# RockingMat/Prot2Text-V2-esm3

Hardware: AMD Instinct MI355X
Metric: contrastive-step samples/sec (protein-text pairs) (higher is better)
Workload: dtype bf16; 1 GPU; cfg3: esm2_t36_3B + Llama-3.1-8B-Instruct (text layers 1-16), per-GPU batch 16 x 1024 residues / 16 x 128 text tokens, readout mix, InfoNCE tau=0.05, adapter fwd+bwd + clip + AdamW, train mode (dropout 0.3), segments 1; global_batch=16, parallelism=dp1 (single process, no collective), streams=text tower and encoder segments on separate HIP streams

## Files before the change

### prot2text-v2-esm3_amd/csrc/gemm_mfma.hip

```cpp
#include <atomic>
#include <type_traits>

#include "common.h"
#include "epilogue.h"
#include "gemm_tile_common.h"
#include "kernels.h"

namespace p2t {

typedef __bf16 bf16x8 __attribute__((ext_vector_type(8)));
using gptr_t = const __attribute__((address_space(1))) void*;
using lptr_t = __attribute__((address_space(3))) void*;

template <int MT, typename Epi, int MODE = TILE_FULL>
__device__ __forceinline__ void gemm_tile(char* smem, const bf16_t* __restrict__ A, int64_t lda, const bf16_t* __restrict__ W,
                                          int64_t ldw, int64_t M, int N, int k0, int ns, int64_t m0, int n0, int n_cover,
                                          const EpiParams& ep, const SplitFix* fix = nullptr, int fix_tile = 0) {
    constexpr int WN = 4, NT = 4, BM = 2 * MT * 16, BN = 256;
    constexpr int AI = BM / 128;
    constexpr int SLOT = (BM + BN) * 64;

    const int lane = threadIdx.x & 63;
    const int w = __builtin_amdgcn_readfirstlane(threadIdx.x >> 6);
    const int wm = w / WN, wn = w % WN;
// ... 333 lines not shown
            tile_coords(n_items + t, n_items + n_tail, tiles_m, tiles_n, tm, tn);
            gemm_tile<8, Epi, TILE_CONSUME>(smem, A, lda, W, ldw, M, N, 0, ns0, (int64_t)tm * 256, tn * 256, n_cover, ep, &fix, t);
        }
    }
}

template <typename Epi>
__global__ void __launch_bounds__(512)
    gemm_nt_mfma_tail_kernel(const bf16_t* __restrict__ A, int64_t lda, const bf16_t* __restrict__ W, int64_t ldw, int64_t M,
                             int N, int K, int tiles_m, int tiles_n, int n_full, int n_tail, int n_cover, EpiParams ep,
                             SplitFix fix) {
    __shared__ __attribute__((aligned(16))) char smem[4 * 512 * 64];
    const int bid = blockIdx.x, ns = K >> 5, ns0 = (ns >> 1) & ~1;
    int tm, tn;
    if (bid < n_full) {
        tile_coords(bid, n_full + n_tail, tiles_m, tiles_n, tm, tn);
        gemm_tile<8, Epi>(smem, A, lda, W, ldw, M, N, 0, ns, (int64_t)tm * 256, tn * 256, n_cover, ep);
    } else if (bid < n_full + n_tail) {
        const int t = bid - n_full;
        tile_coords(n_full + t, n_full + n_tail, tiles_m, tiles_n, tm, tn);
        gemm_tile<8, Epi, TILE_PRODUCE>(smem, A, lda, W, ldw, M, N, ns0 * 32, ns - ns0, (int64_t)tm * 256, tn * 256, n_cover, ep, &fix, t);
    } else {
        const int t = bid - n_full - n_tail;
        tile_coords(n_full + t, n_full + n_tail, tiles_m, tiles_n, tm, tn);
        gemm_tile<8, Epi, TILE_CONSUME>(smem, A, lda, W, ldw, M, N, 0, ns0, (int64_t)tm * 256, tn * 256, n_cover, ep, &fix, t);
    }
}

template <typename Epi>
int launch_gemm_w4_persist(const void* A, int64_t lda, const void* W, int64_t ldw, int64_t M, int N, int K, int n_items, int n_tail, int grid,
                           const EpiParams& ep, const SplitFix& fix, hipStream_t s, int sched = 1);
int launch_gemm_w4(const void* A, int64_t lda, const void* W, int64_t ldw, int64_t M, int N, int K, int n_cover, int out_dtype, int epilogue,
                   const EpiParams& ep, hipStream_t s);
template <typename Epi>
int launch_gemm_w4_pairs(const void* A, int64_t lda, const void* W, int64_t ldw, int64_t M, int N, int K, int n_tail, const EpiParams& ep,
                         const SplitFix& fix, hipStream_t s);
template <typename Epi>
constexpr bool kHasW4Pairs = std::is_same<Epi, EpiResid>::value || std::is_same<Epi, EpiStore<bf16_t>>::value || std::is_same<Epi, EpiStore<float>>::value;
template <typename Epi>
constexpr bool kHasW4 = std::is_same<Epi, EpiStore<bf16_t>>::value || std::is_same<Epi, EpiStore<float>>::value || std::is_same<Epi, EpiResid>::value ||
                        std::is_same<Epi, EpiQkvRope<bf16_t>>::value || std::is_same<Epi, EpiGelu<bf16_t>>::value || std::is_same<Epi, EpiSwiglu<bf16_t>>::value;
template <typename Epi>
constexpr int kW4TileCode = std::is_same<Epi, EpiStore<bf16_t>>::value || std::is_same<Epi, EpiStore<float>>::value ? P2T_EPI_STORE
                            : std::is_same<Epi, EpiResid>::value                                                     ? P2T_EPI_RESID
                            : std::is_same<Epi, EpiGelu<bf16_t>>::value                                              ? P2T_EPI_GELU
                            : std::is_same<Epi, EpiQkvRope<bf16_t>>::value                                           ? P2T_EPI_QKV_ROPE
                                                                                                                      : -1;
template <typename Epi>
constexpr int kW4TileOut = std::is_same<Epi, EpiResid>::value || std::is_same<Epi, EpiStore<float>>::value ? P2T_F32 : P2T_BF16;

struct EpiTraits {
    bool rmw;
    bool w4;
    bool w4_pairs;
    bool w4_tile;
};
template <typename Epi>
constexpr EpiTraits kEpiTraits = {Epi::kRmw, kHasW4<Epi>, kHasW4Pairs<Epi>,
                                  std::is_same<Epi, EpiQkvRope<bf16_t>>::value || std::is_same<Epi, EpiStore<bf16_t>>::value};

GemmFacts gemm_facts(int64_t M, int N, int K, int n_cover, int64_t lda, int64_t ldw, int cus, size_t fix_bytes) {
    GemmFacts f;
    f.M = M; f.lda = lda; f.ldw = ldw; f.N = N; f.K = K; f.n_cover = n_cover; f.cus = cus; f.fix_bytes = fix_bytes;
    f.ns = K >> 5;
    f.tn = ceil_div(n_cover, 256);
    f.items = ceil_div(M, 256) * f.tn;
    f.rem = f.items % cus;
    f.whole_tiles = M % 256 == 0 && N % 256 == 0 && n_cover == N;
    f.stride32 = (int64_t)256 * (lda > ldw ? lda : ldw) * 2 < ((int64_t)1 << 32);
    return f;
}

bool small_tiles_pay(const GemmFacts& f) {
    const double cost256 = (double)ceil_div(f.items, f.cus);
    const double cost128 = (double)ceil_div(ceil_div(f.M, 128) * f.tn, f.cus) * 0.625 * 1.08;
    return cost256 > cost128;
}

static std::atomic<int> g_gemm_policy{0};
void set_gemm_policy(int policy) { g_gemm_policy.store(policy, std::memory_order_relaxed); }
int get_gemm_policy() { return g_gemm_policy.load(std::memory_order_relaxed); }

constexpr size_t kFixHeader = 2048, kFixSlab = 256 * 256 * sizeof(float);
size_t gemm_fix_workspace_bytes() { return kFixHeader + 128 * kFixSlab; }
size_t gemm_fix_header_bytes() { return kFixHeader; }

static bool fix_fits(const GemmFacts& f, int64_t n_tiles) { return f.fix_bytes >= kFixHeader + (size_t)n_tiles * kFixSlab; }

static SplitFix split_fix(void* fix_ws, unsigned fix_epoch) {
    SplitFix f{};
    f.flag = (unsigned*)fix_ws;
    f.timeout = fault_word_ptr();
    f.slab = (float*)((char*)fix_ws + kFixHeader);
    f.epoch = fix_epoch;
    return f;
}


static bool persist_fits(const GemmFacts& f) { return f.whole_tiles && f.items >= f.cus && (f.ns & 3) == 0 && f.ns >= 12; }

static bool persist_pays(const GemmFacts& f, const EpiTraits& t) {
    return persist_fits(f) && (f.rem == 0 || f.ns >= 128 || f.items >= 4 * f.cus || t.rmw);
}

static GemmPlan persist8(const GemmFacts& f, bool pairs, bool halves) {
    GemmPlan p{GEMM_PERSIST, f.cus, f.items};
    if (f.rem == 0 || 2 * f.rem > f.cus || f.rem > 128) return p;
    pairs = pairs && (f.ns & 7) == 0 && fix_fits(f, f.rem);
    if (pairs || halves) {
        p.n_full = f.items - f.rem;
        p.n_tail = f.rem;
        p.half_tail = !pairs;
    }
    return p;
}

static GemmPlan persist4(const GemmFacts& f, bool pairs, int sched = 1) {
    const int64_t t = pairs && f.rem > 0 && 2 * f.rem <= f.cus && fix_fits(f, f.rem) ? f.rem : 0;
    const int64_t n = f.items - t;
    return {GEMM_W4_PERSIST, n < f.cus ? n : f.cus, n, t, 0, sched};
}

static GemmPlan per_tile8(const GemmFacts& f, bool rows128) {
    const int64_t g = rows128 ? ceil_div(f.M, 128) * f.tn : f.items;
    return {rows128 ? GEMM_TILE128 : GEMM_TILE256, g, g};
}

static bool pairs_pay(const GemmFacts& f) { return f.ns >= 192; }

static GemmPlan plan_persist(const GemmFacts& f, const EpiTraits& t, bool no_w4) {
    if (t.w4 && !no_w4 && f.stride32) return persist4(f, pairs_pay(f));
    return persist8(f, pairs_pay(f), true);
}

static GemmPlan plan_per_tile(const GemmFacts& f, const EpiTraits& t, bool no_w4) {
    const int64_t items = f.items;
    if (t.w4_tile && !no_w4 && f.whole_tiles && items < f.cus && items * 4 >= f.cus * 3 && f.K % 128 == 0 && f.K >= 256 && f.stride32)
        return {GEMM_W4_TILE, items, items};
    const bool half_round_long_k = items * 2 <= f.cus && items * 8 >= f.cus * 3 && f.K >= 8192 && fix_fits(f, items);
    if (t.w4_pairs && !no_w4 && f.whole_tiles && half_round_long_k && f.K % 128 == 0 && f.stride32) return {GEMM_W4_PAIRS, 2 * items, 0, items};
    if (half_round_long_k) return {GEMM_SPLITK, 2 * items, 0, items};
    if (small_tiles_pay(f)) return per_tile8(f, true);
    const int64_t n_full = (items / f.cus) * f.cus, n_tail = items - n_full;
    if (n_full > 0 && n_tail > 0 && n_tail <= 128 && (f.ns >= 128 || (f.ns >= 64 && n_full >= 4 * f.cus)) && fix_fits(f, n_tail))
        return {GEMM_SPLITK, n_full + 2 * n_tail, n_full, n_tail};
    return per_tile8(f, false);
}

static GemmPlan plan_default(const GemmFacts& f, const EpiTraits& t, bool no_w4) {
    return persist_pays(f, t) ? plan_persist(f, t, no_w4) : plan_per_tile(f, t, no_w4);
}

#ifdef P2T_LAB
#include "../../tools/lab/gemm_forms_lab.h"
#endif

template <typename Epi>
static GemmPlan plan_shape(const GemmFacts& f, int policy) {
#ifdef P2T_LAB
    if (policy != 0 && policy != 9) return plan_lab<Epi>(f, policy);
#endif
    return plan_default(f, kEpiTraits<Epi>, policy == 9);
}

static int policy_cus() {
#ifdef P2T_LAB
// ... 92 lines not shown
```

### prot2text-v2-esm3_amd/csrc/gemm_tile_common.h

```cpp
#pragma once
#include "common.h"
#include <type_traits>

#include "epilogue.h"

namespace p2t {

struct SplitFix {
    float* slab;
    unsigned* flag;
    unsigned* timeout;
    unsigned epoch;
};
enum { TILE_FULL = 0, TILE_PRODUCE = 1, TILE_CONSUME = 2 };


__device__ __forceinline__ void tile_coords(int id, int n_items, int tiles_m, int tiles_n, int& tm, int& tn) {
    const int q8 = n_items >> 3, r8 = n_items & 7, xcd = id & 7;
    const int swz_id = (xcd < r8 ? xcd * (q8 + 1) : r8 * (q8 + 1) + (xcd - r8) * q8) + (id >> 3);
    constexpr int GM = 4;
    const int band = swz_id / (GM * tiles_n), first_m = band * GM;
    const int gm = min(GM, tiles_m - first_m);
    const int in_band = swz_id - band * GM * tiles_n;
    tm = first_m + in_band % gm;
    tn = in_band / gm;
}

template <int MT, typename Epi, bool INTERIOR = false, bool ADD = false>
__device__ __forceinline__ void tile_epilogue(const f32x4 (&acc)[4][MT], const EpiParams& ep, int64_t M, int N, int n_cover,
                                              int64_t m0, int n0, int wm, int wn, int fr, int kg, const float4* addend = nullptr,
                                              int add_stride = 0, float poison = 0.f) {
    const int nb = n0 + wn * 64 + kg * 8;
    if (!INTERIOR && nb >= n_cover) return;
    float b0[8], b1[8];
#pragma unroll
    for (int e = 0; e < 8; ++e) b0[e] = b1[e] = 0.f;
    if (ep.bias) {
        if (INTERIOR || nb < N) loadW<8>(ep.bias + nb, b0);
        if (INTERIOR || nb + 32 < N) loadW<8>(ep.bias + nb + 32, b1);
    }
    if constexpr (INTERIOR && Epi::kRmw && MT % 4 == 0 && !ADD) {
#pragma unroll
        for (int jb = 0; jb < MT; jb += 4) {
            float r0[4][8], r1[4][8];
#pragma unroll
            for (int jj = 0; jj < 4; ++jj) Epi::template fetch2<8>(ep, m0 + wm * MT * 16 + (jb + jj) * 16 + fr, nb, r0[jj], r1[jj]);
#pragma unroll
            for (int jj = 0; jj < 4; ++jj) {
                const int j = jb + jj;
                const float v0[8] = {acc[0][j][0], acc[0][j][1], acc[0][j][2], acc[0][j][3], acc[1][j][0], acc[1][j][1], acc[1][j][2], acc[1][j][3]};
                const float v1[8] = {acc[2][j][0], acc[2][j][1], acc[2][j][2], acc[2][j][3], acc[3][j][0], acc[3][j][1], acc[3][j][2], acc[3][j][3]};
                Epi::template apply2_fetched<8>(ep, m0 + wm * MT * 16 + j * 16 + fr, nb, v0, v1, b0, b1, r0[jj], r1[jj]);
            }
        }
    } else {
#pragma unroll
        for (int j = 0; j < MT; ++j) {
            const int64_t m = m0 + wm * MT * 16 + j * 16 + fr;
            if (!INTERIOR && m >= M) continue;
            float v0[8] = {acc[0][j][0], acc[0][j][1], acc[0][j][2], acc[0][j][3], acc[1][j][0], acc[1][j][1], acc[1][j][2], acc[1][j][3]};
            float v1[8] = {acc[2][j][0], acc[2][j][1], acc[2][j][2], acc[2][j][3], acc[3][j][0], acc[3][j][1], acc[3][j][2], acc[3][j][3]};
            if constexpr (ADD) {
                const float4 p0 = addend[(0 * MT + j) * add_stride], p1 = addend[(1 * MT + j) * add_stride];
                const float4 p2 = addend[(2 * MT + j) * add_stride], p3 = addend[(3 * MT + j) * add_stride];
                v0[0] += p0.x + poison; v0[1] += p0.y + poison; v0[2] += p0.z + poison; v0[3] += p0.w + poison;
                v0[4] += p1.x + poison; v0[5] += p1.y + poison; v0[6] += p1.z + poison; v0[7] += p1.w + poison;
                v1[0] += p2.x + poison; v1[1] += p2.y + poison; v1[2] += p2.z + poison; v1[3] += p2.w + poison;
                v1[4] += p3.x + poison; v1[5] += p3.y + poison; v1[6] += p3.z + poison; v1[7] += p3.w + poison;
            }
            Epi::template apply2<8, INTERIOR>(ep, m, nb, v0, v1, b0, b1);
        }
    }
}

template <typename Epi, typename = void> struct epi_has_fetch_shared : std::false_type {};
template <typename Epi> struct epi_has_fetch_shared<Epi, std::void_t<decltype(&Epi::fetch_shared)>> : std::true_type {};
template <typename Epi, typename = void> struct epi_has_fetch : std::false_type {};
template <typename Epi> struct epi_has_fetch<Epi, std::void_t<decltype(Epi::kFetch)>> : std::true_type {};
#define P2T_EPI_PIN_GROUP(h, j) \
    asm volatile("" : "+a"(acc[h][0][j]), "+a"(acc[h][1][j]), "+a"(acc[h][2][j]), "+a"(acc[h][3][j])::"memory");
template <int MT, typename Epi, int P = 4>
__device__ __forceinline__ void tile_epilogue_pair(f32x4 (&acc)[2][4][MT], const EpiParams& ep, int64_t m0, int n0, int wm, int wn, int fr, int kg) {
    const int nb0 = n0 + wn * 128 + kg * 8;
    float b[2][2][8];
#pragma unroll
    for (int h = 0; h < 2; ++h)
#pragma unroll
        for (int e = 0; e < 8; ++e) b[h][0][e] = b[h][1][e] = 0.f;
    if (ep.bias) {
#pragma unroll
        for (int h = 0; h < 2; ++h) {
            loadW<8>(ep.bias + nb0 + h * 64, b[h][0]);
            loadW<8>(ep.bias + nb0 + h * 64 + 32, b[h][1]);
        }
    }
    const int64_t mrow = m0 + wm * MT * 16 + fr;
    if constexpr (epi_has_fetch_shared<Epi>::value && P > 0) {
        if (Epi::fetch_shared(ep)) {
            constexpr int PS = P < MT ? P : MT;
            float r[PS][2][8];
#pragma unroll
            for (int u = 0; u < PS; ++u)
#pragma unroll
                for (int e = 0; e < 8; ++e) r[u][0][e] = r[u][1][e] = 0.f;
#pragma unroll
            for (int u = 0; u < PS; ++u) Epi::template fetch2<8, true>(ep, mrow + u * 16, nb0, r[u][0], r[u][1]);
            __builtin_amdgcn_sched_barrier(0);
#pragma unroll
            for (int u = 0; u < MT; ++u) {
                float s0[8], s1[8];
#pragma unroll
                for (int e = 0; e < 8; ++e) { s0[e] = r[u % PS][0][e]; s1[e] = r[u % PS][1][e]; }
                __builtin_amdgcn_sched_barrier(0);
                if (u + PS < MT) Epi::template fetch2<8, true>(ep, mrow + (u + PS) * 16, nb0, r[u % PS][0], r[u % PS][1]);
                __builtin_amdgcn_sched_barrier(0);
#pragma unroll
                for (int h = 0; h < 2; ++h) {
                    P2T_EPI_PIN_GROUP(h, u)
                    const float v0[8] = {acc[h][0][u][0], acc[h][0][u][1], acc[h][0][u][2], acc[h][0][u][3], acc[h][1][u][0], acc[h][1][u][1], acc[h][1][u][2], acc[h][1][u][3]};
                    const float v1[8] = {acc[h][2][u][0], acc[h][2][u][1], acc[h][2][u][2], acc[h][2][u][3], acc[h][3][u][0], acc[h][3][u][1], acc[h][3][u][2], acc[h][3][u][3]};
                    Epi::template apply2_fetched<8, true>(ep, mrow + u * 16, nb0 + h * 64, v0, v1, b[h][0], b[h][1], s0, s1);
                    __builtin_amdgcn_sched_barrier(0);
                }
            }
            return;
        }
    }
    if constexpr ((Epi::kRmw || epi_has_fetch<Epi>::value) && P > 0) {
        constexpr int G = 2 * MT;
        float r[P][2][8];
        if constexpr (!Epi::kRmw) {
#pragma unroll
            for (int g = 0; g < P; ++g)
#pragma unroll
                for (int e = 0; e < 8; ++e) r[g][0][e] = r[g][1][e] = 0.f;
        }
#pragma unroll
        for (int g = 0; g < P; ++g) Epi::template fetch2<8, true>(ep, mrow + (g % MT) * 16, nb0 + (g / MT) * 64, r[g][0], r[g][1]);
        __builtin_amdgcn_sched_barrier(0);
#pragma unroll
        for (int g = 0; g < G; ++g) {
            const int h = g / MT, j = g % MT;
            P2T_EPI_PIN_GROUP(h, j)
            const float v0[8] = {acc[h][0][j][0], acc[h][0][j][1], acc[h][0][j][2], acc[h][0][j][3], acc[h][1][j][0], acc[h][1][j][1], acc[h][1][j][2], acc[h][1][j][3]};
            const float v1[8] = {acc[h][2][j][0], acc[h][2][j][1], acc[h][2][j][2], acc[h][2][j][3], acc[h][3][j][0], acc[h][3][j][1], acc[h][3][j][2], acc[h][3][j][3]};
            float s0[8], s1[8];
#pragma unroll
            for (int e = 0; e < 8; ++e) { s0[e] = r[g % P][0][e]; s1[e] = r[g % P][1][e]; }
            __builtin_amdgcn_sched_barrier(0);
            if (g + P < G) Epi::template fetch2<8, true>(ep, mrow + ((g + P) % MT) * 16, nb0 + ((g + P) / MT) * 64, r[g % P][0], r[g % P][1]);
            __builtin_amdgcn_sched_barrier(0);
            Epi::template apply2_fetched<8, true>(ep, mrow + j * 16, nb0 + h * 64, v0, v1, b[h][0], b[h][1], s0, s1);
            __builtin_amdgcn_sched_barrier(0);
        }
    } else {
#pragma unroll
        for (int h = 0; h < 2; ++h)
#pragma unroll
            for (int j = 0; j < MT; ++j) {
                P2T_EPI_PIN_GROUP(h, j)
                const float v0[8] = {acc[h][0][j][0], acc[h][0][j][1], acc[h][0][j][2], acc[h][0][j][3], acc[h][1][j][0], acc[h][1][j][1], acc[h][1][j][2], acc[h][1][j][3]};
                const float v1[8] = {acc[h][2][j][0], acc[h][2][j][1], acc[h][2][j][2], acc[h][2][j][3], acc[h][3][j][0], acc[h][3][j][1], acc[h][3][j][2], acc[h][3][j][3]};
                Epi::template apply2<8, true>(ep, mrow + j * 16, nb0 + h * 64, v0, v1, b[h][0], b[h][1]);
                __builtin_amdgcn_sched_barrier(0);
            }
    }
}

}
```

### prot2text-v2-esm3_amd/csrc/gemm_w4.hip

```cpp
#include <type_traits>

#include "common.h"
#include "epilogue.h"
#include "gemm_tile_common.h"
#include "kernels.h"

namespace p2t {
#ifdef P2T_LAB
__device__ uint64_t* g_lab_stamp_ptr = nullptr;
#endif

typedef __bf16 bf16x8 __attribute__((ext_vector_type(8)));

template <typename Epi, bool PERSIST, int SCHED = 1, bool PAIRS_ONLY = false>
__global__ void __launch_bounds__(256)
    gemm_nt_w4_kernel(const bf16_t* __restrict__ A, int64_t lda, const bf16_t* __restrict__ W, int64_t ldw, int64_t M, int N, int K,
                      int tiles_m, int tiles_n, int n_items, int n_tail, int n_cover, EpiParams ep, SplitFix fix) {
    constexpr int MT = 8, NT = 8, BUF = 512 * 128, WOFF = 256 * 128, NL = 16;
#ifndef P2T_LAB
    static_assert(SCHED == 1, "the product library carries one instruction order of the K loop; order 0 is in the lab build");
#endif
    constexpr int kEpiOps = 2 * MT * Epi::kMinOps;
    constexpr int kIssuedBeforeWait = SCHED == 0 ? 6 : 9;
    constexpr int kExtCount = kIssuedBeforeWait + kEpiOps > 63 ? 63 : kIssuedBeforeWait + kEpiOps;
// ... 102 lines not shown
            P2T_W4_R0W(0) P2T_W4_PAIR(F, wb, xb, 4) P2T_W4_R0W(1) P2T_W4_PAIR(F, wb, xb, 5) P2T_W4_R0X(0) P2T_W4_GPAIR(9, F, wb, xb, 6) P2T_W4_R0W(2) P2T_W4_PAIR(F, wb, xb, 7)
            P2T_W4_R0W(3) P2T_W4_PAIR(F, wb, xb, 8) P2T_W4_R0X(1) P2T_W4_GPAIR(10, F, wb, xb, 9) P2T_W4_R0W(4) P2T_W4_PAIR(F, wb, xb, 10) P2T_W4_R0W(5) P2T_W4_PAIR(F, wb, xb, 11)
            P2T_W4_R0X(2) P2T_W4_GPAIR(11, F, wb, xb, 12) P2T_W4_R0W(6) P2T_W4_PAIR(F, wb, xb, 13) P2T_W4_R0W(7) P2T_W4_PAIR(F, wb, xb, 14) P2T_W4_R0X(3) P2T_W4_GPAIR(12, F, wb, xb, 15)
            P2T_W4_R0X(4) P2T_W4_PAIR(F, wb, xb, 16) P2T_W4_R0X(5) P2T_W4_PAIR(F, wb, xb, 17) P2T_W4_R0X(6) P2T_W4_GPAIR(13, F, wb, xb, 18) P2T_W4_R0X(7) P2T_W4_PAIR(F, wb, xb, 19)
            P2T_W4_PAIR(F, wb, xb, 20) P2T_W4_GPAIR(14, F, wb, xb, 21) P2T_W4_PAIR(F, wb, xb, 22) P2T_W4_PAIR(F, wb, xb, 23)
            P2T_W4_GPAIR(15, F, wb, xb, 24) P2T_W4_PAIR(F, wb, xb, 25) P2T_W4_PAIR(F, wb, xb, 26) P2T_W4_PAIR(F, wb, xb, 27)
            P2T_W4_PAIR(F, wb, xb, 28) P2T_W4_PAIR(F, wb, xb, 29) P2T_W4_PAIR(F, wb, xb, 30) P2T_W4_PAIR(F, wb, xb, 31)
        }
#ifdef P2T_LAB
        else if constexpr (SCHED == 0) {
            P2T_W4_R1W(0) P2T_W4_PAIR(FI, wa, xa, 0) P2T_W4_R1W(1) P2T_W4_PAIR(FI, wa, xa, 1) P2T_W4_R1X(0) P2T_W4_PAIR(FI, wa, xa, 2) P2T_W4_R1W(2) P2T_W4_PAIR(FI, wa, xa, 3)
            P2T_W4_R1W(3) P2T_W4_PAIR(FI, wa, xa, 4) P2T_W4_R1X(1) P2T_W4_PAIR(FI, wa, xa, 5) P2T_W4_R1W(4) P2T_W4_PAIR(FI, wa, xa, 6) P2T_W4_R1W(5) P2T_W4_PAIR(FI, wa, xa, 7)
            P2T_W4_R1X(2) P2T_W4_PAIR(FI, wa, xa, 8) P2T_W4_R1W(6) P2T_W4_PAIR(FI, wa, xa, 9) P2T_W4_R1W(7) P2T_W4_PAIR(FI, wa, xa, 10) P2T_W4_R1X(3) P2T_W4_PAIR(FI, wa, xa, 11)
            P2T_W4_R1X(4) P2T_W4_PAIR(FI, wa, xa, 12) P2T_W4_R1X(5) P2T_W4_PAIR(FI, wa, xa, 13) P2T_W4_R1X(6) P2T_W4_PAIR(FI, wa, xa, 14) P2T_W4_R1X(7) P2T_W4_PAIR(FI, wa, xa, 15)
            P2T_W4_PAIR(FI, wa, xa, 16) P2T_W4_PAIR(FI, wa, xa, 17) P2T_W4_PAIR(FI, wa, xa, 18) P2T_W4_PAIR(FI, wa, xa, 19)
            asm volatile("s_waitcnt lgkmcnt(0)\n\ts_barrier" ::: "memory");
            P2T_W4_GPAIR(0, FI, wa, xa, 20) P2T_W4_PAIR(FI, wa, xa, 21) P2T_W4_GPAIR(1, FI, wa, xa, 22) P2T_W4_PAIR(FI, wa, xa, 23)
            P2T_W4_PAIR(FI, wa, xa, 24) P2T_W4_GPAIR(2, FI, wa, xa, 25) P2T_W4_PAIR(FI, wa, xa, 26) P2T_W4_PAIR(FI, wa, xa, 27)
            P2T_W4_GPAIR(3, FI, wa, xa, 28) P2T_W4_PAIR(FI, wa, xa, 29) P2T_W4_PAIR(FI, wa, xa, 30) P2T_W4_GPAIR(4, FI, wa, xa, 31)
            P2T_W4_PAIR(F, wb, xb, 0) P2T_W4_GPAIR(5, F, wb, xb, 1) P2T_W4_PAIR(F, wb, xb, 2) P2T_W4_PAIR(F, wb, xb, 3)
            P2T_W4_WAIT_NEXT_STAGE
            P2T_W4_R0W(0) P2T_W4_GPAIR(6, F, wb, xb, 4) P2T_W4_R0W(1) P2T_W4_PAIR(F, wb, xb, 5) P2T_W4_R0X(0) P2T_W4_PAIR(F, wb, xb, 6) P2T_W4_R0W(2) P2T_W4_GPAIR(7, F, wb, xb, 7)
            P2T_W4_R0W(3) P2T_W4_PAIR(F, wb, xb, 8) P2T_W4_R0X(1) P2T_W4_PAIR(F, wb, xb, 9) P2T_W4_R0W(4) P2T_W4_GPAIR(8, F, wb, xb, 10) P2T_W4_R0W(5) P2T_W4_PAIR(F, wb, xb, 11)
            P2T_W4_R0X(2) P2T_W4_PAIR(F, wb, xb, 12) P2T_W4_R0W(6) P2T_W4_GPAIR(9, F, wb, xb, 13) P2T_W4_R0W(7) P2T_W4_PAIR(F, wb, xb, 14) P2T_W4_R0X(3) P2T_W4_PAIR(F, wb, xb, 15)
            P2T_W4_R0X(4) P2T_W4_GPAIR(10, F, wb, xb, 16) P2T_W4_R0X(5) P2T_W4_PAIR(F, wb, xb, 17) P2T_W4_R0X(6) P2T_W4_PAIR(F, wb, xb, 18) P2T_W4_R0X(7) P2T_W4_GPAIR(11, F, wb, xb, 19)
            P2T_W4_PAIR(F, wb, xb, 20) P2T_W4_PAIR(F, wb, xb, 21) P2T_W4_GPAIR(12, F, wb, xb, 22) P2T_W4_PAIR(F, wb, xb, 23)
            P2T_W4_PAIR(F, wb, xb, 24) P2T_W4_GPAIR(13, F, wb, xb, 25) P2T_W4_PAIR(F, wb, xb, 26) P2T_W4_PAIR(F, wb, xb, 27)
            P2T_W4_GPAIR(14, F, wb, xb, 28) P2T_W4_PAIR(F, wb, xb, 29) P2T_W4_PAIR(F, wb, xb, 30) P2T_W4_GPAIR(15, F, wb, xb, 31)
        }
#endif
        a_ptr += 128; w_ptr += 128;
#undef P2T_W4_WAIT_NEXT_STAGE
#undef P2T_W4_PAIR
#undef P2T_W4_R1W
#undef P2T_W4_R1X
#undef P2T_W4_R0W
#undef P2T_W4_R0X
#undef P2T_W4_G
#undef P2T_W4_GPAIR
        asm volatile("s_waitcnt lgkmcnt(0)" ::: "memory");
    };
    using I0 = std::integral_constant<int, 0>;
    using I1 = std::integral_constant<int, 1>;

    auto prologue = [&]() {
#pragma unroll
    for (int b = 0; b < 2; ++b) {
#pragma unroll
        for (int q = 0; q < NL; ++q) dma1(q, b);
        a_ptr += 128; w_ptr += 128;
    }
    asm volatile("s_waitcnt vmcnt(%0)\n\ts_barrier" ::"n"(NL) : "memory");
    rd(wa[0], w_addr, std::integral_constant<int, 0>{}); rd(wa[1], w_addr, std::integral_constant<int, 2048>{});
    rd(wa[2], w_addr, std::integral_constant<int, 4096>{}); rd(wa[3], w_addr, std::integral_constant<int, 6144>{});
    rd(wa[4], w_addr, std::integral_constant<int, 8192>{}); rd(wa[5], w_addr, std::integral_constant<int, 10240>{});
    rd(wa[6], w_addr, std::integral_constant<int, 12288>{}); rd(wa[7], w_addr, std::integral_constant<int, 14336>{});
    rd(xa[0], x_addr, std::integral_constant<int, 0>{}); rd(xa[1], x_addr, std::integral_constant<int, 2048>{});
    rd(xa[2], x_addr, std::integral_constant<int, 4096>{}); rd(xa[3], x_addr, std::integral_constant<int, 6144>{});
    rd(xa[4], x_addr, std::integral_constant<int, 8192>{}); rd(xa[5], x_addr, std::integral_constant<int, 10240>{});
    rd(xa[6], x_addr, std::integral_constant<int, 12288>{}); rd(xa[7], x_addr, std::integral_constant<int, 14336>{});
    asm volatile("s_waitcnt lgkmcnt(0)" ::: "memory");
    };
    auto k_loop = [&](f32x4 (&acc)[2][4][MT], int nk_l, bool ext, bool has_next, int64_t nm0, int nn0) {
        stage(acc, I0{}, T{}, F{}, ext, true);
        stage(acc, I1{}, F{}, F{}, false, true);
        for (int s = 2; s + 2 < nk_l; s += 2) {
            stage(acc, I0{}, F{}, F{}, false, true);
            stage(acc, I1{}, F{}, F{}, false, true);
        }
        if (has_next) {
            a_ptr = (const char*)(A + nm0 * lda);
            w_ptr = (const char*)(W + (int64_t)nn0 * ldw);
        }
        stage(acc, I0{}, F{}, T{}, false, has_next);
        stage(acc, I1{}, F{}, T{}, false, has_next);
        asm volatile("s_nop 7\n\ts_nop 7\n\ts_nop 7" ::: "memory");
#pragma unroll
        for (int h = 0; h < 2; ++h)
#pragma unroll
            for (int i = 0; i < 4; ++i)
#pragma unroll
                for (int j = 0; j < MT; ++j) asm volatile("" : "+a"(acc[h][i][j]));
    };
    if constexpr (!PAIRS_ONLY) {
    prologue();
    {
        f32x4 acc[2][4][MT];
        bool ext = false;
#ifdef P2T_LAB
        constexpr bool kDiagEpi = std::is_same<Epi, EpiStore<bf16_t>>::value || std::is_same<Epi, EpiGelu<bf16_t, false>>::value || std::is_same<Epi, EpiResid>::value;
        uint64_t* dbgp = kDiagEpi ? (uint64_t*)ep.z : nullptr;
        if (!dbgp) dbgp = g_lab_stamp_ptr;
        const bool diag = PERSIST && dbgp != nullptr;
        uint64_t d_loop = 0, d_epi = 0, d_gap = 0, d_tiles = 0, d_real = 0, t_end = 0;
        auto now = [&]() -> uint64_t { uint64_t t; asm volatile("s_memtime %0\n\ts_waitcnt lgkmcnt(0)" : "=s"(t)::"memory"); return t; };
        auto now_real = [&]() -> uint64_t { uint64_t t; asm volatile("s_memrealtime %0\n\ts_waitcnt lgkmcnt(0)" : "=s"(t)::"memory"); return t; };
#endif
        for (;;) {
            const int nxt = item + (int)gridDim.x;
            const bool has_next = PERSIST && nxt < n_items;
            int64_t nm0 = 0;
            int nn0 = 0;
            if (has_next) {
                tile_coords(nxt, n_order, tiles_m, tiles_n, tm, tn);
                nm0 = (int64_t)tm * 256;
                nn0 = tn * 256;
            }
#ifdef P2T_LAB
            uint64_t t0 = 0, r0 = 0, t1 = 0;
            if (diag) { t0 = now(); r0 = now_real(); if (ext) d_gap += t0 - t_end; }
#endif
            k_loop(acc, nk, ext, has_next, nm0, nn0);
#ifdef P2T_LAB
            if (diag) { t1 = now(); d_loop += t1 - t0; d_real += now_real() - r0; d_tiles += 1; }
#endif
            if (PERSIST) {
                int fr_e = fr, kg_e = kg;
                asm volatile("" : "+v"(fr_e), "+v"(kg_e));
                tile_epilogue_pair<MT, Epi, (epi_has_fetch<Epi>::value && !Epi::kRmw) ? 2 : 4>(acc, ep, m0, n0, wm, wn, fr_e, kg_e);
            } else {
                const bool interior = m0 + 256 <= M && n0 + 256 <= N && n0 + 256 <= n_cover;
                if (interior) {
                    tile_epilogue<MT, Epi, true>(acc[0], ep, M, N, n_cover, m0, n0, wm, 2 * wn, fr, kg);
                    tile_epilogue<MT, Epi, true>(acc[1], ep, M, N, n_cover, m0, n0, wm, 2 * wn + 1, fr, kg);
                } else {
                    tile_epilogue<MT, Epi, false>(acc[0], ep, M, N, n_cover, m0, n0, wm, 2 * wn, fr, kg);
                    tile_epilogue<MT, Epi, false>(acc[1], ep, M, N, n_cover, m0, n0, wm, 2 * wn + 1, fr, kg);
                }
            }
#ifdef P2T_LAB
            if (diag) {
                t_end = now();
                d_epi += t_end - t1;
                if (!has_next && threadIdx.x == 0) {
                    uint64_t* d = dbgp + (size_t)blockIdx.x * 8;
                    d[0] = d_loop; d[1] = d_epi; d[2] = d_gap; d[3] = d_tiles; d[4] = d_real;
                }
            }
#endif
            if (!has_next) break;
            ext = true;
            item = nxt;
            m0 = nm0;
            n0 = nn0;
        }
    }
    }
    if (PERSIST && (int)blockIdx.x < 2 * n_tail) {
        const bool producer = (int)blockIdx.x < n_tail;
        const int t = producer ? (int)blockIdx.x : (int)blockIdx.x - n_tail;
        const int nk0 = (nk >> 1) & ~1;
        tile_coords(n_items + t, n_order, tiles_m, tiles_n, tm, tn);
        m0 = (int64_t)tm * 256;
        n0 = tn * 256;
        a_ptr = (const char*)(A + m0 * lda + (producer ? nk0 * 64 : 0));
        w_ptr = (const char*)(W + (int64_t)n0 * ldw + (producer ? nk0 * 64 : 0));
        asm volatile("s_waitcnt vmcnt(0) lgkmcnt(0)\n\ts_barrier" ::: "memory");
        prologue();
        f32x4 acc2[2][4][MT];
        k_loop(acc2, producer ? nk - nk0 : nk0, false, false, 0, 0);
        if (producer) {
            float4* slab = reinterpret_cast<float4*>(fix.slab) + (int64_t)t * (64 * 256) + threadIdx.x;
#pragma unroll
            for (int h = 0; h < 2; ++h)
#pragma unroll
                for (int i = 0; i < 4; ++i)
#pragma unroll
                    for (int j = 0; j < MT; ++j)
                        slab[((h * 4 + i) * MT + j) * 256] = make_float4(acc2[h][i][j][0], acc2[h][i][j][1], acc2[h][i][j][2], acc2[h][i][j][3]);
            asm volatile("s_waitcnt vmcnt(0)" ::: "memory");
            __syncthreads();
            if (w == 0) {
                __builtin_amdgcn_fence(__ATOMIC_RELEASE, "agent");
                asm volatile("s_waitcnt vmcnt(0)" ::: "memory");
                __hip_atomic_store(fix.flag + t, fix.epoch, __ATOMIC_RELAXED, __HIP_MEMORY_SCOPE_AGENT);
            }
        } else {
            {
                const unsigned* fp = fix.flag + t;
                unsigned seen, spins, vtmp;
                const unsigned zero = 0;
                asm volatile(
                    "s_mov_b32 %1, 0\n"
                    "1:\n\t"
                    "global_load_dword %2, %5, %3 sc1\n\t"
                    "s_waitcnt vmcnt(0)\n\t"
                    "v_readfirstlane_b32 %0, %2\n\t"
                    "s_cmp_eq_u32 %0, %4\n\t"
                    "s_cbranch_scc1 2f\n\t"
                    "s_sleep 8\n\t"
                    "s_add_u32 %1, %1, 1\n\t"
                    "s_cmp_lt_u32 %1, 0x400000\n\t"
                    "s_cbranch_scc1 1b\n"
                    "2:\n\t"
                    "buffer_inv sc1"
                    : "=&s"(seen), "=&s"(spins), "=&v"(vtmp)
                    : "s"(fp), "s"(fix.epoch), "v"(zero)
                    : "memory", "scc");
                if (seen != fix.epoch) __hip_atomic_store(fix.timeout, 1u, __ATOMIC_RELAXED, __HIP_MEMORY_SCOPE_AGENT);
            }
            const bool timed_out = __hip_atomic_load(fix.timeout, __ATOMIC_RELAXED, __HIP_MEMORY_SCOPE_AGENT) != 0u;
            const float poison = timed_out ? __builtin_nanf("") : 0.f;
            const float4* slab = reinterpret_cast<const float4*>(fix.slab) + (int64_t)t * (64 * 256) + threadIdx.x;
            tile_epilogue<MT, Epi, true, true>(acc2[0], ep, M, N, n_cover, m0, n0, wm, 2 * wn, fr, kg, slab, 256, poison);
            tile_epilogue<MT, Epi, true, true>(acc2[1], ep, M, N, n_cover, m0, n0, wm, 2 * wn + 1, fr, kg, slab + 4 * MT * 256, 256, poison);
        }
    }
}

template <typename Epi>
static int launch_w4(const void* A, int64_t lda, const void* W, int64_t ldw, int64_t M, int N, int K, int n_cover, const EpiParams& ep,
                     hipStream_t s) {
    const int tiles_m = (int)ceil_div(M, 256), tiles_n = (int)ceil_div(n_cover, 256);
    gemm_nt_w4_kernel<Epi, false><<<dim3((unsigned)(tiles_m * tiles_n)), 256, 0, s>>>((const bf16_t*)A, lda, (const bf16_t*)W, ldw, M, N, K, tiles_m,
                                                                                     tiles_n, tiles_m * tiles_n, 0, n_cover, ep, SplitFix{});
    P2T_LAUNCH_CHECK();
    return P2T_OK;
}

template <typename Epi>
int launch_gemm_w4_persist(const void* A, int64_t lda, const void* W, int64_t ldw, int64_t M, int N, int K, int n_items, int n_tail, int grid,
                           const EpiParams& ep, const SplitFix& fix, hipStream_t s, int sched) {
    const dim3 g((unsigned)(grid < n_items ? grid : n_items));
#ifdef P2T_LAB
    if (sched == 0) {
        gemm_nt_w4_kernel<Epi, true, 0><<<g, 256, 0, s>>>((const bf16_t*)A, lda, (const bf16_t*)W, ldw, M, N, K, (int)(M / 256), N / 256, n_items, n_tail, N, ep, fix);
        P2T_LAUNCH_CHECK();
        return P2T_OK;
    }
#endif
    P2T_REQUIRE(sched == 1, "gemm (four-wave): instruction order %d is not in this build", sched);
    gemm_nt_w4_kernel<Epi, true, 1><<<g, 256, 0, s>>>((const bf16_t*)A, lda, (const bf16_t*)W, ldw, M, N, K, (int)(M / 256), N / 256, n_items, n_tail, N, ep, fix);
    P2T_LAUNCH_CHECK();
    return P2T_OK;
}
template <typename Epi>
int launch_gemm_w4_pairs(const void* A, int64_t lda, const void* W, int64_t ldw, int64_t M, int N, int K, int n_tail, const EpiParams& ep,
                         const SplitFix& fix, hipStream_t s) {
    gemm_nt_w4_kernel<Epi, true, 1, true><<<dim3((unsigned)(2 * n_tail)), 256, 0, s>>>((const bf16_t*)A, lda, (const bf16_t*)W, ldw, M, N, K, (int)(M / 256),
                                                                                      N / 256, 0, n_tail, N, ep, fix);
    P2T_LAUNCH_CHECK();
    return P2T_OK;
}
template int launch_gemm_w4_pairs<EpiResid>(const void*, int64_t, const void*, int64_t, int64_t, int, int, int, const EpiParams&, const SplitFix&, hipStream_t);
template int launch_gemm_w4_pairs<EpiStore<bf16_t>>(const void*, int64_t, const void*, int64_t, int64_t, int, int, int, const EpiParams&, const SplitFix&, hipStream_t);
template int launch_gemm_w4_pairs<EpiStore<float>>(const void*, int64_t, const void*, int64_t, int64_t, int, int, int, const EpiParams&, const SplitFix&, hipStream_t);

template int launch_gemm_w4_persist<EpiStore<bf16_t>>(const void*, int64_t, const void*, int64_t, int64_t, int, int, int, int, int, const EpiParams&, const SplitFix&, hipStream_t, int);
template int launch_gemm_w4_persist<EpiStore<float>>(const void*, int64_t, const void*, int64_t, int64_t, int, int, int, int, int, const EpiParams&, const SplitFix&, hipStream_t, int);
template int launch_gemm_w4_persist<EpiResid>(const void*, int64_t, const void*, int64_t, int64_t, int, int, int, int, int, const EpiParams&, const SplitFix&, hipStream_t, int);
template int launch_gemm_w4_persist<EpiQkvRope<bf16_t>>(const void*, int64_t, const void*, int64_t, int64_t, int, int, int, int, int, const EpiParams&, const SplitFix&, hipStream_t, int);
template int launch_gemm_w4_persist<EpiGelu<bf16_t>>(const void*, int64_t, const void*, int64_t, int64_t, int, int, int, int, int, const EpiParams&, const SplitFix&, hipStream_t, int);
template int launch_gemm_w4_persist<EpiSwiglu<bf16_t>>(const void*, int64_t, const void*, int64_t, int64_t, int, int, int, int, int, const EpiParams&, const SplitFix&, hipStream_t, int);

int launch_gemm_w4(const void* A, int64_t lda, const void* W, int64_t ldw, int64_t M, int N, int K, int n_cover, int out_dtype, int epilogue,
                   const EpiParams& ep, hipStream_t s) {
    if (K % 128 != 0 || K < 256 || M < 1 || (int64_t)256 * (lda > ldw ? lda : ldw) * 2 >= (int64_t)1 << 32) return P2T_ERR_UNSUPPORTED;
    const bool ob = out_dtype == P2T_BF16;
    switch (epilogue) {
        case P2T_EPI_STORE: return ob ? launch_w4<EpiStore<bf16_t>>(A, lda, W, ldw, M, N, K, n_cover, ep, s) : launch_w4<EpiStore<float>>(A, lda, W, ldw, M, N, K, n_cover, ep, s);
        case P2T_EPI_GELU: if (ob) return launch_w4<EpiGelu<bf16_t>>(A, lda, W, ldw, M, N, K, n_cover, ep, s); break;
        case P2T_EPI_RESID: return launch_w4<EpiResid>(A, lda, W, ldw, M, N, K, n_cover, ep, s);
        case P2T_EPI_QKV_ROPE: if (ob) return launch_w4<EpiQkvRope<bf16_t>>(A, lda, W, ldw, M, N, K, n_cover, ep, s); break;
        default: break;
    }
    return P2T_ERR_UNSUPPORTED;
}

}

#ifdef P2T_LAB
extern "C" int p2t_lab_set_stamp_buffer(void* ptr) {
    uint64_t* p = (uint64_t*)ptr;
    return (int)hipMemcpyToSymbol(HIP_SYMBOL(p2t::g_lab_stamp_ptr), &p, sizeof(p));
}
#endif
```

Baseline: 162.4 samples/s.

## Use per-wave split-K fixup flags and a pipelined pair epilogue for tail tiles

In the persistent w4 GEMM's split-K tail, each wave of the writing block now publishes its partial slab with its own flag. This removes the block-wide __syncthreads and the single-wave release fence. The consuming block uses a new tile_epilogue_pair_add, which issues residual fetches before spinning on the flag and then software-pipelines slab loads across row groups. Partial stores use sc1 global stores directly from AGPRs. The finer per-wave handoff depends on the new flag layout (4 words per tile) fitting the header, and relaxed ordering without a fence adds a memory-ordering risk.

```diff
diff --git a/prot2text-v2-esm3_amd/csrc/gemm_mfma.hip b/prot2text-v2-esm3_amd/csrc/gemm_mfma.hip
--- a/prot2text-v2-esm3_amd/csrc/gemm_mfma.hip
+++ b/prot2text-v2-esm3_amd/csrc/gemm_mfma.hip
@@ -439,6 +439,7 @@
 int get_gemm_policy() { return g_gemm_policy.load(std::memory_order_relaxed); }
 
 constexpr size_t kFixHeader = 2048, kFixSlab = 256 * 256 * sizeof(float);
+static_assert(kFixHeader == kFixHeaderBytes && kFixSlab == kFixSlabQuads * 16 && 4 * kFixMaxTail * sizeof(unsigned) == kFixHeader, "split_fix_layout.h");
 size_t gemm_fix_workspace_bytes() { return kFixHeader + 128 * kFixSlab; }
 size_t gemm_fix_header_bytes() { return kFixHeader; }
 
diff --git a/prot2text-v2-esm3_amd/csrc/gemm_tile_common.h b/prot2text-v2-esm3_amd/csrc/gemm_tile_common.h
--- a/prot2text-v2-esm3_amd/csrc/gemm_tile_common.h
+++ b/prot2text-v2-esm3_amd/csrc/gemm_tile_common.h
@@ -3,6 +3,7 @@
 #include <type_traits>
 
 #include "epilogue.h"
+#include "split_fix_layout.h"
 
 namespace p2t {
 
@@ -167,4 +168,121 @@
     }
 }
 
-}
+template <int MT, typename Epi, int P, typename Acquire>
+__device__ __forceinline__ void tile_epilogue_pair_add(f32x4 (&acc)[2][4][MT], const EpiParams& ep, int64_t m0, int n0, int wm, int wn, int fr, int kg,
+                                                       const float4* slab, int stride, Acquire&& acquire) {
+    static_assert(P > 0 && P <= MT, "groups in flight");
+    const int nb0 = n0 + wn * 128 + kg * 8;
+    float b[2][2][8];
+#pragma unroll
+    for (int h = 0; h < 2; ++h)
+#pragma unroll
+        for (int e = 0; e < 8; ++e) b[h][0][e] = b[h][1][e] = 0.f;
+    if (ep.bias) {
+#pragma unroll
+        for (int h = 0; h < 2; ++h) {
+            loadW<8>(ep.bias + nb0 + h * 64, b[h][0]);
+            loadW<8>(ep.bias + nb0 + h * 64 + 32, b[h][1]);
+        }
+    }
+    const int64_t mrow = m0 + wm * MT * 16 + fr;
+    constexpr bool FETCH = Epi::kRmw || epi_has_fetch<Epi>::value;
+#define P2T_EPI_ADD_GROUP(h, j, S)                                                                                                          \
+    P2T_EPI_PIN_GROUP(h, j)                                                                                                                 \
+    const float v0[8] = {acc[h][0][j][0] + (S[0].x + poison), acc[h][0][j][1] + (S[0].y + poison), acc[h][0][j][2] + (S[0].z + poison),    \
+                         acc[h][0][j][3] + (S[0].w + poison), acc[h][1][j][0] + (S[1].x + poison), acc[h][1][j][1] + (S[1].y + poison),    \
+                         acc[h][1][j][2] + (S[1].z + poison), acc[h][1][j][3] + (S[1].w + poison)};                                        \
+    const float v1[8] = {acc[h][2][j][0] + (S[2].x + poison), acc[h][2][j][1] + (S[2].y + poison), acc[h][2][j][2] + (S[2].z + poison),    \
+                         acc[h][2][j][3] + (S[2].w + poison), acc[h][3][j][0] + (S[3].x + poison), acc[h][3][j][1] + (S[3].y + poison),    \
+                         acc[h][3][j][2] + (S[3].z + poison), acc[h][3][j][3] + (S[3].w + poison)};
+    if constexpr (epi_has_fetch_shared<Epi>::value) {
+        if (Epi::fetch_shared(ep)) {
+            float r[P][2][8];
+            float4 s[P][2][4];
+#pragma unroll
+            for (int u = 0; u < P; ++u)
+#pragma unroll
+                for (int e = 0; e < 8; ++e) r[u][0][e] = r[u][1][e] = 0.f;
+#pragma unroll
+            for (int u = 0; u < P; ++u) Epi::template fetch2<8, true>(ep, mrow + u * 16, nb0, r[u][0], r[u][1]);
+            const float poison = acquire();
+#pragma unroll
+            for (int u = 0; u < P; ++u)
+#pragma unroll
+                for (int h = 0; h < 2; ++h)
+#pragma unroll
+                    for (int i = 0; i < 4; ++i) s[u][h][i] = slab[((h * 4 + i) * MT + u) * stride];
+            __builtin_amdgcn_sched_barrier(0);
+#pragma unroll
+            for (int u = 0; u < MT; ++u) {
+                float s0[8], s1[8];
+#pragma unroll
+                for (int e = 0; e < 8; ++e) { s0[e] = r[u % P][0][e]; s1[e] = r[u % P][1][e]; }
+                float4 q[2][4];
+#pragma unroll
+                for (int h = 0; h < 2; ++h)
+#pragma unroll
+                    for (int i = 0; i < 4; ++i) q[h][i] = s[u % P][h][i];
+                __builtin_amdgcn_sched_barrier(0);
+                if (u + P < MT) {
+#pragma unroll
+                    for (int h = 0; h < 2; ++h)
+#pragma unroll
+                        for (int i = 0; i < 4; ++i) s[u % P][h][i] = slab[((h * 4 + i) * MT + u + P) * stride];
+                    Epi::template fetch2<8, true>(ep, mrow + (u + P) * 16, nb0, r[u % P][0], r[u % P][1]);
+                }
+                __builtin_amdgcn_sched_barrier(0);
+#pragma unroll
+                for (int h = 0; h < 2; ++h) {
+                    P2T_EPI_ADD_GROUP(h, u, q[h])
+                    Epi::template apply2_fetched<8, true>(ep, mrow + u * 16, nb0 + h * 64, v0, v1, b[h][0], b[h][1], s0, s1);
+                    __builtin_amdgcn_sched_barrier(0);
+                }
+            }
+            return;
+        }
+    }
+    constexpr int G = 2 * MT;
+    float r[FETCH ? P : 1][2][8];
+    float4 s[P][4];
+    if constexpr (FETCH) {
+        if constexpr (!Epi::kRmw) {
+#pragma unroll
+            for (int g = 0; g < P; ++g)
+#pragma unroll
+                for (int e = 0; e < 8; ++e) r[g][0][e] = r[g][1][e] = 0.f;
+        }
+#pragma unroll
+        for (int g = 0; g < P; ++g) Epi::template fetch2<8, true>(ep, mrow + g * 16, nb0, r[g][0], r[g][1]);
+    }
+    const float poison = acquire();
+#pragma unroll
+    for (int g = 0; g < P; ++g)
+#pragma unroll
+        for (int i = 0; i < 4; ++i) s[g][i] = slab[(i * MT + g) * stride];
+    __builtin_amdgcn_sched_barrier(0);
+#pragma unroll
+    for (int g = 0; g < G; ++g) {
+        const int h = g / MT, j = g % MT;
+        P2T_EPI_ADD_GROUP(h, j, s[g % P])
+        float s0[8], s1[8];
+        if constexpr (FETCH) {
+#pragma unroll
+            for (int e = 0; e < 8; ++e) { s0[e] = r[g % P][0][e]; s1[e] = r[g % P][1][e]; }
+        }
+        __builtin_amdgcn_sched_barrier(0);
+        if (g + P < G) {
+            const int hn = (g + P) / MT, jn = (g + P) % MT;
+#pragma unroll
+            for (int i = 0; i < 4; ++i) s[g % P][i] = slab[((hn * 4 + i) * MT + jn) * stride];
+            if constexpr (FETCH) Epi::template fetch2<8, true>(ep, mrow + jn * 16, nb0 + hn * 64, r[g % P][0], r[g % P][1]);
+        }
+        __builtin_amdgcn_sched_barrier(0);
+        if constexpr (FETCH) Epi::template apply2_fetched<8, true>(ep, mrow + j * 16, nb0 + h * 64, v0, v1, b[h][0], b[h][1], s0, s1);
+        else Epi::template apply2<8, true>(ep, mrow + j * 16, nb0 + h * 64, v0, v1, b[h][0], b[h][1]);
+        __builtin_amdgcn_sched_barrier(0);
+    }
+#undef P2T_EPI_ADD_GROUP
+}
+
+}
diff --git a/prot2text-v2-esm3_amd/csrc/gemm_w4.hip b/prot2text-v2-esm3_amd/csrc/gemm_w4.hip
--- a/prot2text-v2-esm3_amd/csrc/gemm_w4.hip
+++ b/prot2text-v2-esm3_amd/csrc/gemm_w4.hip
@@ -208,19 +208,22 @@
 #pragma unroll
                 for (int j = 0; j < MT; ++j) asm volatile("" : "+a"(acc[h][i][j]));
     };
+#ifdef P2T_LAB
+    constexpr bool kDiagEpi = std::is_same<Epi, EpiStore<bf16_t>>::value || std::is_same<Epi, EpiGelu<bf16_t, false>>::value || std::is_same<Epi, EpiResid>::value;
+    uint64_t* dbgp = kDiagEpi ? (uint64_t*)ep.z : nullptr;
+    if (!dbgp) dbgp = g_lab_stamp_ptr;
+    const bool diag = PERSIST && dbgp != nullptr;
+    uint64_t t_end = 0;
+    auto now = [&]() -> uint64_t { uint64_t t; asm volatile("s_memtime %0\n\ts_waitcnt lgkmcnt(0)" : "=s"(t)::"memory"); return t; };
+    auto now_real = [&]() -> uint64_t { uint64_t t; asm volatile("s_memrealtime %0\n\ts_waitcnt lgkmcnt(0)" : "=s"(t)::"memory"); return t; };
+#endif
     if constexpr (!PAIRS_ONLY) {
     prologue();
     {
         f32x4 acc[2][4][MT];
         bool ext = false;
 #ifdef P2T_LAB
-        constexpr bool kDiagEpi = std::is_same<Epi, EpiStore<bf16_t>>::value || std::is_same<Epi, EpiGelu<bf16_t, false>>::value || std::is_same<Epi, EpiResid>::value;
-        uint64_t* dbgp = kDiagEpi ? (uint64_t*)ep.z : nullptr;
-        if (!dbgp) dbgp = g_lab_stamp_ptr;
-        const bool diag = PERSIST && dbgp != nullptr;
-        uint64_t d_loop = 0, d_epi = 0, d_gap = 0, d_tiles = 0, d_real = 0, t_end = 0;
-        auto now = [&]() -> uint64_t { uint64_t t; asm volatile("s_memtime %0\n\ts_waitcnt lgkmcnt(0)" : "=s"(t)::"memory"); return t; };
-        auto now_real = [&]() -> uint64_t { uint64_t t; asm volatile("s_memrealtime %0\n\ts_waitcnt lgkmcnt(0)" : "=s"(t)::"memory"); return t; };
+        uint64_t d_loop = 0, d_epi = 0, d_gap = 0, d_tiles = 0, d_real = 0;
 #endif
         for (;;) {
             const int nxt = item + (int)gridDim.x;
@@ -259,7 +262,7 @@
                 t_end = now();
                 d_epi += t_end - t1;
                 if (!has_next && threadIdx.x == 0) {
-                    uint64_t* d = dbgp + (size_t)blockIdx.x * 8;
+                    uint64_t* d = dbgp + (size_t)blockIdx.x * 16;
                     d[0] = d_loop; d[1] = d_epi; d[2] = d_gap; d[3] = d_tiles; d[4] = d_real;
                 }
             }
@@ -273,37 +276,52 @@
     }
     }
     if (PERSIST && (int)blockIdx.x < 2 * n_tail) {
-        const bool producer = (int)blockIdx.x < n_tail;
-        const int t = producer ? (int)blockIdx.x : (int)blockIdx.x - n_tail;
+        const bool second = (int)blockIdx.x < n_tail;
+        const int t = second ? (int)blockIdx.x : (int)blockIdx.x - n_tail;
         const int nk0 = (nk >> 1) & ~1;
         tile_coords(n_items + t, n_order, tiles_m, tiles_n, tm, tn);
         m0 = (int64_t)tm * 256;
         n0 = tn * 256;
-        a_ptr = (const char*)(A + m0 * lda + (producer ? nk0 * 64 : 0));
-        w_ptr = (const char*)(W + (int64_t)n0 * ldw + (producer ? nk0 * 64 : 0));
+        a_ptr = (const char*)(A + m0 * lda + (second ? nk0 * 64 : 0));
+        w_ptr = (const char*)(W + (int64_t)n0 * ldw + (second ? nk0 * 64 : 0));
         asm volatile("s_waitcnt vmcnt(0) lgkmcnt(0)\n\ts_barrier" ::: "memory");
         prologue();
         f32x4 acc2[2][4][MT];
-        k_loop(acc2, producer ? nk - nk0 : nk0, false, false, 0, 0);
-        if (producer) {
-            float4* slab = reinterpret_cast<float4*>(fix.slab) + (int64_t)t * (64 * 256) + threadIdx.x;
+#ifdef P2T_LAB
+        uint64_t tk0 = 0, tk1 = 0;
+        if (diag) tk0 = now();
+#endif
+        k_loop(acc2, second ? nk - nk0 : nk0, false, false, 0, 0);
+#ifdef P2T_LAB
+        if (diag) tk1 = now();
+#endif
+        int keep_s = second ? 0 : 1;
+        asm volatile("" : "+v"(keep_s));
+        const bool keep = __builtin_amdgcn_readfirstlane(keep_s) != 0;
+        unsigned* const fp = fix.flag + fix_flag_word_w4(t, w);
+        if (!keep) {
+            const char* sbase = (const char*)(reinterpret_cast<const float4*>(fix.slab) + fix_slab_quad0(t));
+            const uint32_t svoff = threadIdx.x * 16u;
 #pragma unroll
             for (int h = 0; h < 2; ++h)
 #pragma unroll
                 for (int i = 0; i < 4; ++i)
 #pragma unroll
                     for (int j = 0; j < MT; ++j)
-                        slab[((h * 4 + i) * MT + j) * 256] = make_float4(acc2[h][i][j][0], acc2[h][i][j][1], acc2[h][i][j][2], acc2[h][i][j][3]);
+                        asm volatile("global_store_dwordx4 %0, %1, %2 sc1" ::"v"(svoff), "a"(acc2[h][i][j]), "s"(sbase + ((h * 4 + i) * MT + j) * 4096) : "memory");
             asm volatile("s_waitcnt vmcnt(0)" ::: "memory");
-            __syncthreads();
-            if (w == 0) {
-                __builtin_amdgcn_fence(__ATOMIC_RELEASE, "agent");
-                asm volatile("s_waitcnt vmcnt(0)" ::: "memory");
-                __hip_atomic_store(fix.flag + t, fix.epoch, __ATOMIC_RELAXED, __HIP_MEMORY_SCOPE_AGENT);
+            __hip_atomic_store(fp, fix.epoch, __ATOMIC_RELAXED, __HIP_MEMORY_SCOPE_AGENT);
+#ifdef P2T_LAB
+            if (diag) {
+                const uint64_t tp = now();
+                if (lane == 0 && wn == 0) dbgp[(size_t)blockIdx.x * 16 + 12] = tp - tk1;
             }
+#endif
         } else {
-            {
-                const unsigned* fp = fix.flag + t;
+#ifdef P2T_LAB
+            uint64_t ts = 0;
+#endif
+            auto acquire = [&]() __attribute__((always_inline)) -> float {
                 unsigned seen, spins, vtmp;
                 const unsigned zero = 0;
                 asm volatile(
@@ -321,15 +339,28 @@
                     "2:\n\t"
                     "buffer_inv sc1"
                     : "=&s"(seen), "=&s"(spins), "=&v"(vtmp)
-                    : "s"(fp), "s"(fix.epoch), "v"(zero)
+                    : "s"((const unsigned*)fp), "s"(fix.epoch), "v"(zero)
                     : "memory", "scc");
                 if (seen != fix.epoch) __hip_atomic_store(fix.timeout, 1u, __ATOMIC_RELAXED, __HIP_MEMORY_SCOPE_AGENT);
+#ifdef P2T_LAB
+                if (diag) ts = now();
+#endif
+                const bool timed_out = __hip_atomic_load(fix.timeout, __ATOMIC_RELAXED, __HIP_MEMORY_SCOPE_AGENT) != 0u;
+                return timed_out ? __builtin_nanf("") : 0.f;
+            };
+            const float4* slab = reinterpret_cast<const float4*>(fix.slab) + fix_slab_quad0(t) + threadIdx.x;
+            int fr_e = fr, kg_e = kg;
+            asm volatile("" : "+v"(fr_e), "+v"(kg_e));
+            tile_epilogue_pair_add<MT, Epi, (epi_has_fetch<Epi>::value && !Epi::kRmw) ? 2 : 4>(acc2, ep, m0, n0, wm, wn, fr_e, kg_e, slab, 256, acquire);
+#ifdef P2T_LAB
+            if (diag) {
+                const uint64_t td = now();
+                if (lane == 0 && wn == 0) {
+                    uint64_t* d = dbgp + (size_t)blockIdx.x * 16;
+                    d[8] = tk1 - tk0; d[9] = ts - tk1; d[10] = td - ts; d[11] = t_end ? tk0 - t_end : 0;
+                }
             }
-            const bool timed_out = __hip_atomic_load(fix.timeout, __ATOMIC_RELAXED, __HIP_MEMORY_SCOPE_AGENT) != 0u;
-            const float poison = timed_out ? __builtin_nanf("") : 0.f;
-            const float4* slab = reinterpret_cast<const float4*>(fix.slab) + (int64_t)t * (64 * 256) + threadIdx.x;
-            tile_epilogue<MT, Epi, true, true>(acc2[0], ep, M, N, n_cover, m0, n0, wm, 2 * wn, fr, kg, slab, 256, poison);
-            tile_epilogue<MT, Epi, true, true>(acc2[1], ep, M, N, n_cover, m0, n0, wm, 2 * wn + 1, fr, kg, slab + 4 * MT * 256, 256, poison);
+#endif
         }
     }
 }
diff --git a/prot2text-v2-esm3_amd/csrc/split_fix_layout.h b/prot2text-v2-esm3_amd/csrc/split_fix_layout.h
--- /dev/null
+++ b/prot2text-v2-esm3_amd/csrc/split_fix_layout.h
@@ -0,0 +1,14 @@
+#pragma once
+#if defined(__HIPCC__) || defined(__CUDACC__)
+#define P2T_HD __host__ __device__
+#else
+#define P2T_HD
+#endif
+
+namespace p2t {
+constexpr int kFixHeaderBytes = 2048;
+constexpr int kFixMaxTail = 128;
+constexpr int kFixSlabQuads = 64 * 256;
+P2T_HD constexpr int fix_flag_word_w4(int t, int w) { return 4 * t + w; }
+P2T_HD constexpr long long fix_slab_quad0(int t) { return (long long)t * kFixSlabQuads; }
+}
```

New measurement: 163.5 samples/s, median of 6. No clear change (+0.7%).
